# pku-lab-1806-llm/lab-1806-vec-db

Hardware: AMD Instinct MI355X
Metric: queries/sec at recall@10, Gist1M d=960 (Flat brute force, L2Sqr, k=10) (higher is better)
Workload: dtype f32 (int8 lower-bound filter pass); 1 GPU; flat_knn_gist1m; rows=1000000, dim=960, k=10, dist=L2Sqr, parallelism=single GPU, steps_in_flight=1, queries_per_corpus_pass=128

## Files before the change

lab_1806_vec_db_amd/csrc/api.hip:

```cpp
#include <algorithm>
#include <cmath>
#include <cstring>

#include "ctx.hpp"
#include "pq_hnsw.hpp"

using namespace vdb;

static thread_local std::string g_last_error;
void vdb::set_last_error(const std::string &m) { g_last_error = m; }
void vdb::require_gpu() {
    int cnt = 0;
    hipError_t e = hipGetDeviceCount(&cnt);
    if (e != hipSuccess || cnt <= 0)
        throw Error(VDB_ERR_NOGPU, std::string("no usable HIP device (libvdbhip has no CPU fallback): ") +
                                       hipGetErrorString(e));
}

void vdb::merge_topk_dev(Index &ix, const void *d_dists, const void *d_ids, const void *d_counts, uint64_t stride_d,
                           uint64_t stride_i, uint64_t stride_c, uint64_t n_shards, uint64_t nq, uint64_t k,
                           void *d_out_idx, void *d_out_dist, void *d_out_count, void *stream) {
    VDB_REQUIRE(d_dists && d_ids && d_counts && d_out_idx && d_out_dist && d_out_count, "null argument");
    VDB_REQUIRE(k >= 1 && k <= 1024, "k must be in 1..1024");
    VDB_REQUIRE(nq <= 65535 && n_shards <= 65535, "too many queries or shards for one call");
// ... 536 lines not shown
    else if (n == "flat_gemm_tw")
        gemm_set_tw((int)value);
    else if (n == "flat_gemm_nt")
        gemm_set_nt((int)value);
    else if (n == "flat_gemm_zigzag")
        gemm_set_zigzag((int)value);
    else if (n == "flat_gemm_block_rows") {
        VDB_REQUIRE(value >= 0, "flat_gemm_block_rows must be >= 0");
        gemm_set_block_rows((uint64_t)value);
    }
    else if (n == "flat_gemm_stagger")
        gemm_set_stagger((int)value);
    else if (n == "flat_gemm_debug")
        idx->ix.flat_gemm_debug = (int)value;
    else if (n == "flat_tail")
        idx->ix.flat_tail_mode = (int)value;
    else if (n == "flat_tail_lb_nw")
        flat_tail_lb_set_nw((int)value);
    else if (n == "flat_small")
        idx->ix.flat_small_mode = (int)value;
    else if (n == "flat_small_max_rows")
        idx->ix.flat_small_max_rows = (uint64_t)value;
    else if (n == "flat_half")
        idx->ix.flat_half_mode = (int)value;
    else if (n == "flat_i8")
        idx->ix.flat_i8_mode = (int)value;
    else if (n == "flat_i8_rows") {
        VDB_REQUIRE(value >= 64 && value <= 8192 && value % 64 == 0, "flat_i8_rows must be a multiple of 64 in [64, 8192]");
        idx->ix.flat_i8_kprime = (uint32_t)value;
    }
    else if (n == "flat_range_max_results") {
        VDB_REQUIRE(value >= 0, "flat_range_max_results must be >= 0");
        idx->ix.range_max_results = (uint64_t)value;
    }
    else if (n == "debug_alloc_fail_over")
        devbuf_fail_over() = (size_t)value;
    else if (n == "flat_i8_unit_min")
        idx->ix.flat_i8_unit_min = (int)value;
    else if (n == "flat_i8_full")
        idx->ix.flat_i8_full = (int)value;
    else if (n == "flat_i8_refine") {
        idx->ix.flat_i8_refine = (int)value;
        idx->ix.i8_refine_on = 0;
        idx->ix.i8_refine_calls = 0;
    }
    else if (n == "flat_i8_second")
        idx->ix.flat_i8_second = (int)value;
    else if (n == "flat_i8_stats") {
        idx->ix.flat_i8_stats = (int)value;
        for (auto &h : idx->ix.i8_rounds_hist) h = 0;
        idx->ix.i8_hits_sum = 0;
        idx->ix.i8_hits_max = 0;
        idx->ix.i8_stat_queries = 0;
    }
    else if (n == "flat_i8_hits") {
        VDB_REQUIRE(value >= 256 && value <= 4096, "flat_i8_hits must be in [256, 4096]");
        idx->ix.flat_i8_hits = (uint32_t)value;
    }
    else if (n == "flat_gemm8_sample_res")
        gemm8_set_sample_res((int)value);
    else if (n == "flat_gemm8_nt")
        gemm8_set_nt((int)value);
    else if (n == "flat_gemm8_kc")
        gemm8_set_kc((int)value);
    else if (n == "flat_gemm8_burst")
        gemm8_set_burst((int)value);
    else if (n == "flat_gemm8_res")
        gemm8_set_res((int)value);
    else if (n == "flat_gemm8_coop")
        gemm8_set_coop((int)value);
    else if (n == "flat_gemm8_grid")
        gemm8_set_grid((int)value);
    else if (n == "flat_gemm_coop")
        gemm_set_coop((int)value);
    else if (n == "flat_half_kmul") {
        VDB_REQUIRE(value >= 1 && value <= 64, "flat_half_kmul must be in [1, 64]");
        idx->ix.flat_half_kmul = (uint32_t)value;
    }
    else
        throw Error(VDB_ERR_INVALID, "unknown parameter " + n);
    VDB_API_END
}
int vdb_index_prepare(vdb_index *idx, int all_tiers) {
    VDB_API_BEGIN
    VDB_REQUIRE(idx, "null index");
    require_gpu();
    idx->ix.prepare_flat(all_tiers != 0);
    VDB_API_END
}
int vdb_flat_fallback_count(const vdb_index *idx, uint64_t *out) {
    VDB_API_BEGIN
    VDB_REQUIRE(idx && out, "null argument");
    *out = idx->ix.fallback_count.load();
    VDB_API_END
}

int vdb_get_stat(const vdb_index *idx, const char *name, uint64_t *out) {
    VDB_API_BEGIN
    VDB_REQUIRE(idx && name && out, "null argument");
    std::string n(name);
    if (n == "flat_fallback")
        *out = idx->ix.fallback_count.load();
    else if (n == "flat_half_queries")
        *out = idx->ix.half_queries.load();
    else if (n == "flat_half_redo")
        *out = idx->ix.half_redo.load();
    else if (n == "flat_half_valid")
        *out = idx->ix.half_m.valid ? 1 : 0;
    else if (n == "flat_gemm_coop_sets")
        *out = gemm_last_coop();
    else if (n == "flat_gemm8_coop_sets")
        *out = gemm8_last_coop();
    else if (n == "flat_i8_queries")
        *out = idx->ix.i8_queries.load();
    else if (n == "flat_i8_redo")
        *out = idx->ix.i8_redo.load();
    else if (n == "flat_i8_valid")
        *out = idx->ix.i8_m.valid ? 1 : 0;
    else if (n == "flat_range_queries")
        *out = idx->ix.range_queries.load();
    else if (n == "flat_range_i8_queries")
        *out = idx->ix.range_i8_queries.load();
    else if (n == "flat_range_scan_queries")
        *out = idx->ix.range_scan_queries.load();
    else if (n == "flat_range_hits")
        *out = idx->ix.range_hits.load();
    else if (n == "flat_range_hits_max")
        *out = idx->ix.range_hits_max.load();
    else if (n == "flat_range_results")
        *out = idx->ix.range_results.load();
    else if (n.rfind("flat_i8_rounds_", 0) == 0 && n.size() == 16 && n[15] >= '0' && n[15] <= '8')
        *out = idx->ix.i8_rounds_hist[n[15] - '0'].load();
    else if (n == "mirror_alloc_failures")
        *out = idx->ix.mirror_alloc_failures.load();
    else if (n == "flat_i8_second_queries")
        *out = idx->ix.i8_second_queries.load();
    else if (n == "flat_i8_second_redo")
        *out = idx->ix.i8_second_redo.load();
    else if (n == "flat_i8_hits_sum")
        *out = idx->ix.i8_hits_sum.load();
    else if (n == "flat_i8_hits_max")
        *out = idx->ix.i8_hits_max.load();
    else if (n == "flat_i8_stat_queries")
        *out = idx->ix.i8_stat_queries.load();
    else if (n == "flat_i8_rows_walked")
        *out = idx->ix.i8_rows_walked.load();
    else if (n == "flat_bf16_mirror")
        *out = idx->ix.tiled_built ? 1 : 0;
    else if (n == "hnsw_heap_walk_queries")
        *out = idx->ix.hnsw.heap_walk_queries.load();
    else if (n == "hnsw_half_dropped")
        *out = idx->ix.hnsw.last_half_dropped.load();
    else if (n == "ivf_last_offers")
        *out = idx->ix.ivf.last_offers.load();
    else if (n == "ivf_last_rows_fetched_q8")
        *out = idx->ix.ivf.last_rows_fetched_q8.load();
    else if (n == "ivf_last_kept_q8")
        *out = idx->ix.ivf.last_kept_q8.load();
    else if (n == "ivf_last_kept")
        *out = idx->ix.ivf.last_kept.load();
    else if (n == "pq_adc16_queries")
        *out = idx->ix.pq.adc16_queries.load();
    else if (n == "pq_adc16_redo")
        *out = idx->ix.pq.adc16_redo.load();
    else if (n == "flat_i8_refine_queries")
        *out = idx->ix.i8_refine_queries.load();
    else if (n == "flat_i8_refine_on")
        *out = (uint64_t)idx->ix.i8_refine_on.load();
    else if (n == "pq_q8_overflow")
        *out = idx->ix.pq.q8_overflow.load();
    else if (n == "pq_q8_short")
        *out = idx->ix.pq.q8_short.load();
    else if (n == "pq_q8_hits_sum")
        *out = idx->ix.pq.q8_hits_sum.load();
    else if (n == "pq_q8_hits_max")
        *out = idx->ix.pq.q8_hits_max.load();
    else if (n == "hbm_bytes_per_row")
        *out = idx->ix.hbm_bytes_per_row();
    else
        throw Error(VDB_ERR_INVALID, "unknown statistic " + n);
    VDB_API_END
}

int vdb_pq_attach(vdb_index *idx, uint64_t n_bits, uint64_t m, const float *centroids, const uint8_t *codes) {
    VDB_API_BEGIN
    VDB_REQUIRE(idx && centroids, "null argument");
    pq_attach(idx->ix, n_bits, m, centroids, codes);
    VDB_API_END
}
int vdb_pq_build(vdb_index *idx, uint64_t n_bits, uint64_t m, uint64_t train_n, uint64_t max_iter, float tol,
                 uint64_t seed) {
    VDB_API_BEGIN
    VDB_REQUIRE(idx, "null index");
    pq_build(idx->ix, n_bits, m, train_n, max_iter, tol, seed);
    VDB_API_END
}
int vdb_pq_clear(vdb_index *idx) {
// ... 534 lines not shown
```

lab_1806_vec_db_amd/csrc/index.hip:

```cpp
#include "index.hpp"

#include <algorithm>
#include <cmath>
#include <cstring>

namespace vdb {

Index::Index(int dev, uint64_t d, int ds, bool u8) : device(dev), dim(d), dist(ds), elem_u8(u8) {
#ifndef VDB_HOST_SANITIZER_BUILD
    use_device();
    hipDeviceProp_t prop;
    VDB_HIP(hipGetDeviceProperties(&prop, dev));
    num_cu = prop.multiProcessorCount > 0 ? prop.multiProcessorCount : 256;
    std::string arch = prop.gcnArchName;
    if (arch.rfind("gfx950", 0) != 0)
        throw Error(4, "libvdbhip is built for gfx950 (MI355X) only; device reports " + arch);
#endif
}

std::unique_ptr<Workspace> Index::acquire_ws() {
    use_device();
    {
        std::lock_guard<std::mutex> g(ws_mu);
        if (!ws_free.empty()) {
// ... 605 lines not shown
                                 d_cand, d_hits, CAND_CAP, flat_gemm_debug, num_cu, s,
                                 i8_second ? CAND_CAP : std::max<uint32_t>(64u, s_step * s_rank));
    else if (gemm)
        launch_flat_gemm_filter(xt, n, (uint32_t)dim, ws.qfrag_g.as<float>(), d_qmul, (uint32_t)ngroups,
                                d_sq.as<float>(), cosine, d_tau, d_cand, d_hits, CAND_CAP, flat_gemm_debug, num_cu, s);
    else
        launch_flat_mfma_filter(d_tiled.as<float>(), n, (uint32_t)dim, ws.qfrag.as<float>(), (uint32_t)nbatch,
                                d_sq.as<float>(), cosine, d_tau, d_cand, d_hits, CAND_CAP, d_sync, num_cu, s);
    prof_end(ws);
    {
        std::lock_guard<std::mutex> g(pass_mu);
        if (!pass_ev) VDB_HIP(hipEventCreateWithFlags(&pass_ev, hipEventDisableTiming));
        VDB_HIP(hipEventRecord(pass_ev, s));
        pass_ev_valid = true;
    }
    SplitErr se;
    if (half) {
        se.qerr = d_qerr;
        se.dx_abs = half_dx_abs;
        se.dx_rel = half_dx_rel;
    }
    if (i8) {
        se.qoff = d_qoff;
        se.mu_norm = i8_mu_norm;
    }
    if (i8 || (flat_tail_mode != 1 && !elem_u8 && flat_tail64_supported((uint32_t)dim, kprime, ksel))) {
        FlatTailArgs t{};
        t.cand = d_cand;
        t.cap = CAND_CAP;
        t.cnt = d_hits;
        t.kprime = kprime;
        t.ksel = ksel;
        t.kstride = (uint32_t)k;
        t.X = d_rows.as<float>();
        t.dim = (uint32_t)dim;
        t.Q = d_q;
        t.metric = cosine ? MET_COSINE : MET_L2_DIRECT;
        t.xsq = d_sq.as<float>();
        t.qsq = ws.qsq.as<float>();
        t.n_rows = n;
        t.xsq_max = xsq_max;
        t.xsq_min_pos = xsq_min_pos;
        t.cosine = cosine;
        t.se = se;
        t.id_offset = id_offset;
        bool refine = false;
        if (i8 && !i8_second && nq >= 64 && flat_i8_refine != 1) {
            bool on = flat_i8_refine == 2;
            if (flat_i8_refine == 0 && i8_refine_on.load() != 0) on = (i8_refine_calls.fetch_add(1) % 32u) != 31u;
            refine = on && ensure_rows_h(ws);
        }
        const size_t st_off = (nq + 15) & ~size_t(15);
        const bool want_stats = i8 && flat_i8_stats;
        t.flags = static_cast<uint8_t *>(ws.pinned(want_stats ? st_off + nq * sizeof(uint32_t) : nq));
        if (want_stats) t.qstat = reinterpret_cast<uint32_t *>(t.flags + st_off);
        p.stats = want_stats;
        p.refined = refine;
        if (refine) {
            launch_flat_refine_half(d_rows_h.as<uint16_t>(), (uint32_t)dim, half_sx(), half_dx_abs, half_dx_rel, cosine, d_q, d_sq.as<float>(),
                                    ws.qsq.as<float>(), d_qoff, d_cand, CAND_CAP, d_hits, (uint32_t)nq, CAND_CAP, s);
            i8_refine_queries += nq;
        }
        t.out_idx = d_idx;
        t.out_dist = d_dist;
        t.out_count = d_cnt;
        t.tau = d_tau;
        if (i8 && i8_second && nq <= 96 && flat_i8_full != 1) {
            ws.keys_b.reserve(nq * size_t(CAND_CAP) * sizeof(uint64_t));
            launch_flat_full_lb(t, (uint32_t)nq, ws.keys_b.as<uint64_t>(), ws.keys_c.as<uint64_t>(), s);
        } else if (i8)
            launch_flat_tail_lb(t, (uint32_t)nq, s);
        else
            launch_flat_tail64(t, (uint32_t)nq, s);
    } else {
        launch_topk_merge_counted(d_cand, CAND_CAP, d_hits, (uint32_t)nq, kprime, ws.keys_a.as<uint64_t>(), s);
        rerank_rows((uint32_t)dim, d_q, (uint32_t)nq, cosine ? MET_COSINE : MET_L2_DIRECT, d_sq.as<float>(),
                      ws.qsq.as<float>(), ws.keys_a.as<uint64_t>(), ws.keys_b.as<uint64_t>(), kprime, capp, s);
        launch_topk_merge(ws.keys_b.as<uint64_t>(), 1, capp, (uint32_t)nq, ksel, ws.keys_c.as<uint64_t>(), s);
        launch_flat_finish(ws.keys_c.as<uint64_t>(), capk, ws.keys_a.as<uint64_t>(), capp, (uint32_t)nq, ksel, (uint32_t)k, kprime,
                           n, ws.qsq.as<float>(), xsq_max, xsq_min_pos, cosine, (uint32_t)dim, se, d_hits, CAND_CAP, id_offset,
                           static_cast<uint8_t *>(ws.pinned(nq)), d_idx, d_dist, d_cnt, s);
    }
    p.active = true;
    p.half = half;
    p.i8 = i8;
    p.i8_second = i8_second;
    p.kprime = kprime;
    p.ksel = ksel;
    p.nq = nq;
    p.k = k;
    p.d_q = d_q;
    p.d_idx = d_idx;
    p.d_dist = d_dist;
    p.d_cnt = d_cnt;
}

uint64_t Index::flat_knn_finish(Workspace &ws, FlatPending &p) {
    hipStream_t s = ws.stream;
    if (!p.active) return 0;
    p.active = false;
    const uint64_t nq = p.nq, k = p.k;
    const uint8_t *flags = static_cast<const uint8_t *>(ws.pinned(nq));
    VDB_SYNC(s);
    std::vector<uint64_t> redo;
    for (uint64_t q = 0; q < nq; q++)
        if (flags[q] & 1u) redo.push_back(q);
    if (p.half) {
        half_queries += nq;
        half_redo += redo.size();
    }
    if (p.i8 && p.i8_second) {
        i8_second_queries += nq;
        i8_second_redo += redo.size();
    }
    const bool try_second = p.i8 && !p.i8_second && flat_i8_second != 1 && !redo.empty();
    if (p.i8 && !p.i8_second) {
        i8_queries += nq;
        if (!try_second) i8_redo += redo.size();
        if (flat_i8_refine == 0 && nq >= 64) {
            uint64_t rs = 0;
            for (uint64_t q = 0; q < nq; q++) rs += std::min<uint32_t>(flags[q] >> 1, 32u);
            const double mean_rounds = double(rs) / double(nq);
            if (!p.refined) {
                const int was = i8_refine_on.load();
                const int now = was ? (mean_rounds >= 4.0 ? 1 : 0) : (mean_rounds >= 6.0 ? 1 : 0);
                if (now != was) {
                    i8_refine_on = now;
                    i8_refine_calls = 0;
                }
            }
        }
        if (p.stats) {
            const uint32_t *qs = reinterpret_cast<const uint32_t *>(flags + ((nq + 15) & ~size_t(15)));
            uint64_t hs = 0, hm = 0;
            for (uint64_t q = 0; q < nq; q++) {
                const uint32_t r = qs[q] & 0xFFu, h = qs[q] >> 8;
                i8_rounds_hist[r < 8 ? r : 8] += 1;
                hs += h;
                hm = std::max<uint64_t>(hm, h);
            }
            i8_hits_sum += hs;
            i8_stat_queries += nq;
            uint64_t cur = i8_hits_max.load();
            while (hm > cur && !i8_hits_max.compare_exchange_weak(cur, hm)) {
            }
        }
    }
    if (redo.empty()) return 0;
    if (!p.half && !p.i8) fallback_count += redo.size();
    const uint64_t nr = redo.size();
    DevBuf rx, rq, rqs, ri, rd, rc, rdk;
    rx.reserve(nr * sizeof(uint64_t));
    rq.reserve(nr * dim * sizeof(float));
    rqs.reserve(nr * sizeof(float));
    ri.reserve(nr * k * sizeof(uint64_t));
    rd.reserve(nr * k * sizeof(float));
    rc.reserve(nr * sizeof(uint64_t));
    VDB_HIP(hipMemcpyAsync(rx.p, redo.data(), nr * sizeof(uint64_t), hipMemcpyHostToDevice, s));
    launch_gather_rows_f32(p.d_q, rx.as<uint64_t>(), nr, (uint32_t)dim, rq.as<float>(), s);
    launch_gather_rows_f32(ws.qsq.as<float>(), rx.as<uint64_t>(), nr, 1, rqs.as<float>(), s);
    if (try_second) {
        rdk.reserve(nr * sizeof(float));
        launch_gather_dk(p.d_dist, p.d_cnt, rx.as<uint64_t>(), nr, (uint32_t)k, p.ksel, rdk.as<float>(), s);
    }
    VDB_HIP(hipMemsetAsync(ri.p, 0, nr * k * sizeof(uint64_t), s));
    VDB_HIP(hipMemsetAsync(rd.p, 0, nr * k * sizeof(float), s));
    VDB_SYNC(s);
    if (try_second)
        i8_redo += flat_knn_device(ws, rq.as<float>(), nr, k, ri.as<uint64_t>(), rd.as<float>(), rc.as<uint64_t>(), true, 0, true, rdk.as<float>());
    else if (p.i8)
        flat_knn_device(ws, rq.as<float>(), nr, k, ri.as<uint64_t>(), rd.as<float>(), rc.as<uint64_t>(), true, 0, false);
    else if (p.half)
        flat_knn_device(ws, rq.as<float>(), nr, k, ri.as<uint64_t>(), rd.as<float>(), rc.as<uint64_t>(), false, p.kprime);
    else
        flat_exact_device(ws, rq.as<float>(), rqs.as<float>(), nr, p.ksel, k, ri.as<uint64_t>(), rd.as<float>(), rc.as<uint64_t>());
    launch_scatter_results(ri.as<uint64_t>(), rd.as<float>(), rc.as<uint64_t>(), rx.as<uint64_t>(), nr, (uint32_t)k, p.d_idx, p.d_dist, p.d_cnt, s);
    VDB_SYNC(s);
    return p.i8 ? nr : 0;
}

void Index::flat_range_device(Workspace &ws, const float *d_q, uint64_t nq, const float *d_radius, uint64_t limit, RangeResult &out) {
    hipStream_t s = ws.stream;
    out.device = device;
    out.nq = nq;
    out.lims.assign(nq + 1, 0);
    range_queries += nq;
    if (nq == 0) return;
    if (n == 0) {
        range_scan_queries += nq;
        return;
    }
    constexpr uint32_t CAND_CAP = 8192;
    constexpr uint64_t QCH = 1024;
    constexpr uint32_t BQ = 8;
// ... 237 lines not shown
```

lab_1806_vec_db_amd/csrc/index.hpp:

```cpp
#pragma once
#include <algorithm>
#include <atomic>
#include <cmath>
#include <cstdlib>
#include <functional>
#include <map>
#include <memory>
#include <mutex>
#include <string>
#include <vector>

#include "common.hpp"
#include "kernels.hpp"

namespace vdb {

inline bool devbuf_efence() {
    static const bool on = [] {
        const char *e = std::getenv("VDB_EFENCE");
        return e && e[0] == '1';
    }();
    return on;
}
inline std::atomic<size_t> &devbuf_fail_over() {
// ... 224 lines not shown
    size_t elem_size() const { return elem_u8 ? 1 : sizeof(float); }
    const float *rows_f32_view(DevBuf &scratch, uint64_t r0, uint64_t r1, hipStream_t s) const;
    template <class F>
    void for_tile_chunks(Workspace &ws, uint64_t t_begin, uint64_t t_end, uint64_t n_rows, F fn) const {
        if (!elem_u8) {
            fn(d_rows.as<float>(), t_begin, t_end, std::min(t_begin * 16, n_rows), n_rows);
            return;
        }
        constexpr uint64_t CH = 12 * 64;
        ws.dense.reserve(CH * 16 * dim * sizeof(float));
        for (uint64_t t = t_begin; t < t_end; t += CH) {
            const uint64_t tb = std::min(t_end, t + CH), ra = std::min(t * 16, n_rows), rb = std::min(tb * 16, n_rows);
            fn(rows_f32_view(ws.dense, ra, rb, ws.stream), t, tb, ra, rb);
        }
    }
    DevBuf d_rows, d_sq;
    std::atomic<uint64_t> mirror_alloc_failures{0};
    DevBuf d_tiled;
    RowMirror tiled_m{mirror_alloc_failures, {&d_tiled}};
    const std::atomic<bool> &tiled_built = tiled_m.valid;
    bool ensure_tiled(Workspace &ws);
    void prepare_flat(bool all_tiers);
    uint64_t hbm_bytes_per_row() const;
    DevBuf d_tiled_h, d_half_err;
    int half_exp = 0;
    float half_dx_abs = 0.0f, half_dx_rel = 0.0f;
    int flat_half_mode = 0;
    uint32_t flat_half_kmul = 4;
    std::atomic<uint64_t> half_queries{0}, half_redo{0};
    void half_refresh(Workspace &ws, uint64_t n_old, uint64_t n_new);
    RowMirror half_m{mirror_alloc_failures, {&d_tiled_h}};
    bool i8_defers_half() const;
    bool ensure_half(Workspace &ws);
    float half_sx() const { return std::ldexp(1.0f, 13 - half_exp); }
    DevBuf d_tiled_i8, d_rowc_i8, d_mu_i8;
    RowMirror i8_m{mirror_alloc_failures, {&d_tiled_i8, &d_rowc_i8}};
    uint64_t i8_mu_rows = 0;
    float i8_l1 = 0.0f, i8_l2 = 0.0f, i8_mu_norm = 0.0f;
    int flat_i8_mode = 0;
    uint32_t flat_i8_kprime = 2048;
    int flat_i8_full = 0;
    int flat_i8_refine = 0;
    std::atomic<int> i8_refine_on{0};
    std::atomic<uint32_t> i8_refine_calls{0};
    std::atomic<uint64_t> i8_refine_queries{0};
    int flat_i8_unit_min = 0;
    int flat_i8_second = 0;
    std::atomic<uint64_t> i8_second_queries{0}, i8_second_redo{0};
    uint32_t flat_i8_hits = 1024;
    std::atomic<uint64_t> i8_queries{0}, i8_redo{0};
    int flat_i8_stats = 0;
    std::atomic<uint64_t> i8_rounds_hist[9] = {};
    std::atomic<uint64_t> i8_hits_sum{0}, i8_hits_max{0}, i8_stat_queries{0};
    std::atomic<uint64_t> i8_rows_walked{0};
    bool i8_applicable(uint32_t ksel) const;
    bool i8_mirror_applicable() const;
    bool ensure_i8(Workspace &ws);
    void build_i8(Workspace &ws);
    DevBuf d_rows_h;
    RowMirror rows_h_m{mirror_alloc_failures, {&d_rows_h}};
    int rows_h_exp = 0;
    bool ensure_rows_h(Workspace &ws);
    DevBuf d_rows_q8, d_q8_scale, d_q8_err;
    RowMirror rows_q8_m{mirror_alloc_failures, {&d_rows_q8, &d_q8_scale, &d_q8_err}};
    bool ensure_rows_q8(Workspace &ws);
    std::vector<float> h_sq;
    float xsq_max = 0.0f;
    float xsq_min_pos = 3.4e38f;
    mutable std::vector<float> h_rows;
    mutable bool host_valid = true;
    mutable std::mutex host_mu;
    int flat_mode = 0;
    int flat_gemm_mode = 0;
    int flat_gemm_debug = 0;
    int flat_tail_mode = 0;
    int flat_small_mode = 0;
    uint64_t flat_small_max_rows = 16384;
    bool flat_small_applies(uint64_t nq, uint64_t k) const;
    void flat_small_device(Workspace &ws, const float *q, uint64_t nq, uint64_t k, uint64_t *o_idx, float *o_dist, uint64_t *o_cnt);
    std::atomic<uint64_t> fallback_count{0};
    PQState pq;
    HNSWState hnsw;
    IVFState ivf;

    std::mutex ws_mu;
    std::vector<std::unique_ptr<Workspace>> ws_free;
    std::mutex pass_mu;
    hipEvent_t pass_ev = nullptr;
    bool pass_ev_valid = false;
    bool prof_on = false;
    std::mutex prof_mu;
    std::map<std::string, ProfEntry> prof;

    Index(int dev, uint64_t d, int ds, bool u8 = false);
    ~Index() {
        if (pass_ev) (void)hipEventDestroy(pass_ev);
    }
    void use_device() const {
#ifndef VDB_HOST_SANITIZER_BUILD
        VDB_HIP(hipSetDevice(device));
#endif
    }
    std::unique_ptr<Workspace> acquire_ws();
    void release_ws(std::unique_ptr<Workspace> ws);
    const float *host_rows() const;

// ... 40 lines not shown
```

lab_1806_vec_db_amd/csrc/k_exact.hip:

```cpp
#include <algorithm>
#include <atomic>
#include <cstdio>
#include <cstdlib>
#include <vector>

#include "common.hpp"
#include "kernels.hpp"

#pragma clang fp contract(off)

namespace vdb {

enum Fold : int { FOLD_L2 = 0, FOLD_DOT = 1 };

template <int FOLD>
__device__ __forceinline__ float fold1(float acc, float x, float q) {
    if (FOLD == FOLD_L2) {
        float df = x - q;
        float sq = df * df;
        return acc + sq;
    } else {
        float p = x * q;
        return acc + p;
    }
// ... 747 lines not shown
        a.out_idx[uint64_t(q) * a.kstride + lane] = ok ? uint64_t(uint32_t(sorted)) + a.id_offset : 0;
        a.out_dist[uint64_t(q) * a.kstride + lane] = ok ? f32_from_orderable(uint32_t(sorted >> 32)) : 0.0f;
    }
    const uint32_t count = __builtin_popcountll(__ballot(ok));
    if (lane == 0) {
        if (a.out_count) a.out_count[q] = count;
        a.flags[q] = flag;
    }
}
bool flat_tail64_supported(uint32_t dim, uint32_t kprime, uint32_t ksel) {
    return (dim & 3) == 0 && dim >= 64 && dim <= 8192 && kprime >= 1 && kprime <= 64 && ksel >= 1 && ksel <= 64;
}
void launch_flat_tail64(const FlatTailArgs &a, uint32_t nq, hipStream_t s) {
    if (nq == 0) return;
    VDB_REQUIRE(flat_tail64_supported(a.dim, a.kprime, a.ksel), "flat_tail64: unsupported shape");
    const size_t lds = (size_t(a.dim / 4) + 4 * 72) * sizeof(float4);
    if (a.metric == MET_L2_DIRECT)
        hipLaunchKernelGGL((k_flat_tail64<FOLD_L2>), dim3(nq), dim3(256), lds, s, a);
    else
        hipLaunchKernelGGL((k_flat_tail64<FOLD_DOT>), dim3(nq), dim3(256), lds, s, a);
    VDB_HIP(hipGetLastError());
}

#define TAIL_LB_AUTO_NW(nq) 40
template <int NW>
__device__ __forceinline__ uint64_t block_top64_above(const uint64_t *__restrict__ src, uint32_t total, uint64_t (*sbest)[64], uint64_t above) {
    const uint32_t lane = threadIdx.x & 63, wave = threadIdx.x >> 6;
    const uint32_t batches = (total + 255) / 256;
    uint64_t best = PAIR_NONE;
    for (uint32_t bt = wave; bt < batches; bt += NW) {
        uint64_t r[4];
#pragma unroll
        for (int u = 0; u < 4; u++) {
            const uint32_t i = (bt * 4 + u) * 64 + lane;
            const uint64_t v = i < total ? src[i] : PAIR_NONE;
            r[u] = v > above ? v : PAIR_NONE;
        }
        const uint64_t tau = __shfl(best, 63);
        uint64_t lo = r[0] < r[1] ? r[0] : r[1], lo2 = r[2] < r[3] ? r[2] : r[3];
        lo = lo < lo2 ? lo : lo2;
        if (__ballot(lo < tau) == 0) continue;
        bitonic_sort_from<2, 4>(r, lane);
        const uint64_t a = merge64(r[0], r[1], lane), b = merge64(r[2], r[3], lane);
        best = merge64(best, merge64(a, b, lane), lane);
    }
    sbest[wave][lane] = best;
    __syncthreads();
    if (wave != 0) return PAIR_NONE;
    uint64_t m = sbest[0][lane];
#pragma unroll
    for (int w = 1; w < NW; w++) m = merge64(m, sbest[w][lane], lane);
    return m;
}
__device__ __forceinline__ uint8_t flat_certify_lb(uint64_t ek, float kappa, uint32_t q, const FlatTailArgs &a) {
    if (ek == PAIR_NONE) return 1;
    const float dk = f32_from_orderable(uint32_t(ek >> 32));
    return flat_lb_excludes(dk, kappa, a.qsq[q], a.se.qoff[q], a.cosine, a.xsq_max, a.xsq_min_pos, a.se.mu_norm, a.dim) ? 0 : 1;
}
template <int FOLD, int NW, int PCD>
__global__ __launch_bounds__(NW * 64, PCD ? 4 : 1) void k_flat_tail_lb(FlatTailArgs a) {
    constexpr bool PC = PCD != 0;
    static_assert(NW == 8 || NW == 4 || NW == 2 || NW == 1, "a stage covers the 64 keys of a round");
    static_assert(!PC || NW == 4, "producer / consumer fold: four waves");
    constexpr int RW = 64 / NW, NP = RW / 8;
    constexpr int DEPTH = PC ? PCD : (NW == 8 ? 8 : (NW == 4 ? 4 : (NW == 2 ? 3 : 2)));
    extern __shared__ float4 ftl_smem[];
    __shared__ uint64_t sbest[NW][64];
    __shared__ uint64_t skeys[64];
    __shared__ uint32_t s_flag;
    const uint32_t q = blockIdx.x, lane = threadIdx.x & 63, wave = threadIdx.x >> 6;
    const uint32_t d4 = a.dim / 4;
    float4 *qs4 = ftl_smem, *tile = ftl_smem + d4 + wave * (RW * 9);
    for (uint32_t i = threadIdx.x; i < d4; i += NW * 64) qs4[i] = reinterpret_cast<const float4 *>(a.Q + uint64_t(q) * a.dim)[i];
    const uint32_t cnt_q = a.cnt[q];
    const uint32_t total = cnt_q <= a.cap ? cnt_q : 0;
    const uint32_t kk = a.ksel;
    const float tau_q = a.tau[q];
    uint64_t run = PAIR_NONE;
    uint64_t above = 0;
    uint8_t flag = 1;
    const uint32_t rounds = cnt_q <= a.cap ? a.kprime / 64 : 0;
#ifdef VDB_TAIL_STAMPS
    uint32_t ns = 0;
#define TAIL_STAMP()                                                                                      \
    do {                                                                                                  \
        if (a.stamps && threadIdx.x == 0 && ns < 30) a.stamps[q * 32 + ns++] = __builtin_readcyclecounter(); \
    } while (0)
#else
#define TAIL_STAMP() do { } while (0)
#endif
    TAIL_STAMP();
    uint32_t rounds_done = 0;
    for (uint32_t rd = 0; rd < rounds; rd++) {
        rounds_done = rd + 1;
        const uint64_t best = block_top64_above<NW>(a.cand + uint64_t(q) * a.cap, total, sbest, above);
        __syncthreads();
        if (wave == 0) sbest[0][lane] = best;
        if (threadIdx.x < 64) skeys[threadIdx.x] = PAIR_NONE;
        __syncthreads();
        TAIL_STAMP();
        uint32_t idx[NP];
        bool live[NP];
#pragma unroll
        for (int i = 0; i < NP; i++) {
            const uint32_t j = wave * RW + 8 * i + (lane >> 3);
            const uint64_t c = sbest[0][j];
            live[i] = c != PAIR_NONE && j < 63;
            idx[i] = live[i] ? uint32_t(c) : 0u;
#if defined(VDB_TAIL_ABLATE) && VDB_TAIL_ABLATE == 1
            idx[i] &= 63u;
#endif
        }
        float acc;
        if constexpr (PC) {
            const bool consumer = wave == (blockIdx.x & 3u);
            acc = pc_rerank_fold<FOLD, DEPTH>(a.X, a.dim, idx, live, qs4, ftl_smem + d4, wave, lane, consumer);
            const uint64_t c = sbest[0][lane];
            if (consumer && c != PAIR_NONE && lane < 63)
                skeys[lane] = pair_key(FOLD == FOLD_L2 ? acc : epilogue(MET_COSINE, acc, a.xsq[uint32_t(c)], a.qsq[q]), uint32_t(c));
        } else {
            if constexpr (NW == 8)
                acc = group_rerank_fold<FOLD, 8>(a.X, a.dim, idx[0], live[0], qs4, tile, lane);
            else
                acc = group_rerank_fold_n<FOLD, DEPTH, RW>(a.X, a.dim, idx, live, qs4, tile, lane);
            const uint32_t j = wave * RW + lane / NW;
            const uint64_t c = sbest[0][j];
            if (c != PAIR_NONE && j < 63 && lane % NW == 0)
                skeys[j] = pair_key(FOLD == FOLD_L2 ? acc : epilogue(MET_COSINE, acc, a.xsq[uint32_t(c)], a.qsq[q]), uint32_t(c));
        }
        __syncthreads();
        TAIL_STAMP();
        if (wave == 0) {
            run = merge64(run, sort64(skeys[lane], lane), lane);
            const uint64_t ek = __shfl(run, kk - 1), nxt = sbest[0][63];
            if (lane == 0) {
                const float kappa = nxt == PAIR_NONE ? tau_q : f32_from_orderable(uint32_t(nxt >> 32));
                s_flag = flat_certify_lb(ek, kappa, q, a) | (nxt == PAIR_NONE ? 2u : 0u);
            }
        }
        __syncthreads();
        TAIL_STAMP();
        const uint32_t f = s_flag;
        if ((f & 1u) == 0) {
            flag = 0;
            break;
        }
        if (f & 2u) break;
        above = sbest[0][62];
        __syncthreads();
    }
#ifdef VDB_TAIL_STAMPS
    if (a.stamps && threadIdx.x == 0) {
        a.stamps[q * 32 + 30] = ns;
        a.stamps[q * 32 + 31] = total;
    }
#endif
    if (wave != 0) return;
    const bool ok = lane < a.ksel && run != PAIR_NONE;
    if (lane < a.ksel) {
        a.out_idx[uint64_t(q) * a.kstride + lane] = ok ? uint64_t(uint32_t(run)) + a.id_offset : 0;
        a.out_dist[uint64_t(q) * a.kstride + lane] = ok ? f32_from_orderable(uint32_t(run >> 32)) : 0.0f;
    }
    const uint32_t count = __builtin_popcountll(__ballot(ok));
    if (lane == 0) {
        if (a.out_count) a.out_count[q] = count;
        a.flags[q] = uint8_t(flag | ((rounds_done < 127u ? rounds_done : 127u) << 1));
        if (a.qstat) a.qstat[q] = rounds_done | ((cnt_q < 0xFFFFFFu ? cnt_q : 0xFFFFFFu) << 8);
    }
}
bool flat_tail_lb_supported(uint32_t dim, uint32_t kprime, uint32_t ksel) {
    return (dim & 3) == 0 && dim >= 64 && dim <= 8192 && kprime >= 64 && kprime % 64 == 0 && kprime <= 8192 && ksel >= 1 && ksel <= 64;
}
static std::atomic<int> g_tail_lb_nw{0};
void flat_tail_lb_set_nw(int v) { g_tail_lb_nw = v; }
#ifdef VDB_TAIL_STAMPS
static void tail_stamps_report(unsigned long long *d, uint32_t nq, hipStream_t s) {
    VDB_SYNC(s);
    std::vector<unsigned long long> h(size_t(nq) * 32);
    VDB_HIP(hipMemcpy(h.data(), d, h.size() * 8, hipMemcpyDeviceToHost));
    VDB_HIP(hipFree(d));
    uint32_t hist[8] = {0}, nr = 0;
    double sel = 0, fold = 0, cert = 0, life = 0;
    for (uint32_t q = 0; q < nq; q++) {
        const unsigned long long *t = &h[size_t(q) * 32];
        const uint32_t ns = (uint32_t)t[30], r = ns ? (ns - 1) / 3 : 0;
        hist[r < 7 ? r : 7]++;
        if (ns) life += double(t[ns - 1] - t[0]);
        for (uint32_t i = 0; i < r; i++, nr++) {
            sel += double(t[1 + 3 * i] - t[3 * i]);
            fold += double(t[2 + 3 * i] - t[1 + 3 * i]);
            cert += double(t[3 + 3 * i] - t[2 + 3 * i]);
        }
    }
    fprintf(stderr, "TAIL_STAMPS nq %u  queries by rounds 0:%u 1:%u 2:%u 3:%u 4:%u 5+:%u  ticks per round: select %.0f fold %.0f merge+certify %.0f  per workgroup %.0f\n",
            nq, hist[0], hist[1], hist[2], hist[3], hist[4], hist[5] + hist[6] + hist[7], sel / (nr ? nr : 1), fold / (nr ? nr : 1),
            cert / (nr ? nr : 1), life / nq);
}
#endif
void launch_flat_tail_lb(const FlatTailArgs &a0, uint32_t nq, hipStream_t s) {
    if (nq == 0) return;
    FlatTailArgs a = a0;
#ifdef VDB_TAIL_STAMPS
    static std::atomic<int> calls{0};
    const char *want = getenv("VDB_TAIL_STAMPS");
    unsigned long long *stamps = nullptr;
    if (want && ++calls == atoi(want)) {
        VDB_HIP(hipMalloc(&stamps, size_t(nq) * 32 * 8));
        VDB_HIP(hipMemset(stamps, 0, size_t(nq) * 32 * 8));
        a.stamps = stamps;
    }
#endif
    VDB_REQUIRE(flat_tail_lb_supported(a.dim, a.kprime, a.ksel) && (a.metric == MET_L2_DIRECT || a.metric == MET_COSINE) && a.se.qoff && a.tau,
                "flat_tail_lb: unsupported shape");
    VDB_REQUIRE((a.metric == MET_COSINE) == (a.cosine != 0) && (a.metric == MET_L2_DIRECT || (a.xsq && a.qsq)), "flat_tail_lb: metric / norms");
    const size_t lds = (size_t(a.dim / 4) + 2 * 64 * 9) * sizeof(float4);
    int nw = g_tail_lb_nw;
    if (nw != 8 && nw != 4 && nw != 2 && nw != 1 && nw != 40 && nw != 41) nw = TAIL_LB_AUTO_NW(nq);
    if (a.metric == MET_COSINE) {
        if (nw == 8)
            hipLaunchKernelGGL((k_flat_tail_lb<FOLD_DOT, 8, 0>), dim3(nq), dim3(512), lds, s, a);
        else if (nw == 41)
            hipLaunchKernelGGL((k_flat_tail_lb<FOLD_DOT, 4, 5>), dim3(nq), dim3(256), lds, s, a);
        else
            hipLaunchKernelGGL((k_flat_tail_lb<FOLD_DOT, 4, 3>), dim3(nq), dim3(256), lds, s, a);
    } else if (nw == 40)
        hipLaunchKernelGGL((k_flat_tail_lb<FOLD_L2, 4, 3>), dim3(nq), dim3(256), lds, s, a);
    else if (nw == 41)
        hipLaunchKernelGGL((k_flat_tail_lb<FOLD_L2, 4, 5>), dim3(nq), dim3(256), lds, s, a);
    else if (nw == 8)
        hipLaunchKernelGGL((k_flat_tail_lb<FOLD_L2, 8, 0>), dim3(nq), dim3(512), lds, s, a);
    else if (nw == 4)
        hipLaunchKernelGGL((k_flat_tail_lb<FOLD_L2, 4, 0>), dim3(nq), dim3(256), lds, s, a);
    else if (nw == 2)
        hipLaunchKernelGGL((k_flat_tail_lb<FOLD_L2, 2, 0>), dim3(nq), dim3(128), lds, s, a);
    else
        hipLaunchKernelGGL((k_flat_tail_lb<FOLD_L2, 1, 0>), dim3(nq), dim3(64), lds, s, a);
    VDB_HIP(hipGetLastError());
#ifdef VDB_TAIL_STAMPS
    if (stamps) tail_stamps_report(stamps, nq, s);
#endif
}

__global__ __launch_bounds__(64) void k_flat_finish_lb(FlatTailArgs a, const uint64_t *__restrict__ exact_sorted, uint32_t lde) {
    const uint32_t q = blockIdx.x, lane = threadIdx.x;
    const uint32_t cnt_q = a.cnt[q];
    const uint64_t e = lane < a.ksel ? exact_sorted[uint64_t(q) * lde + lane] : PAIR_NONE;
    const uint64_t ek = __shfl(e, a.ksel - 1);
    uint8_t flag = 1;
    if (lane == 0 && cnt_q <= a.cap) flag = flat_certify_lb(ek, a.tau[q], q, a);
    const bool ok = lane < a.ksel && e != PAIR_NONE;
    if (lane < a.ksel) {
        a.out_idx[uint64_t(q) * a.kstride + lane] = ok ? uint64_t(uint32_t(e)) + a.id_offset : 0;
        a.out_dist[uint64_t(q) * a.kstride + lane] = ok ? f32_from_orderable(uint32_t(e >> 32)) : 0.0f;
    }
    const uint32_t count = __builtin_popcountll(__ballot(ok));
    if (lane == 0) {
        if (a.out_count) a.out_count[q] = count;
        a.flags[q] = flag;
        if (a.qstat) a.qstat[q] = 0xFFu | ((cnt_q < 0xFFFFFFu ? cnt_q : 0xFFFFFFu) << 8);
    }
}
void launch_flat_full_lb(const FlatTailArgs &a, uint32_t nq, uint64_t *exact_keys , uint64_t *topk ,
                         hipStream_t s) {
    if (nq == 0) return;
    VDB_REQUIRE(a.ksel >= 1 && a.ksel <= 64 && (a.dim & 3) == 0 && a.se.qoff && a.tau, "flat_full_lb: unsupported shape");
    launch_rerank(a.X, a.dim, a.Q, nq, a.metric, a.xsq, a.qsq, a.cand, exact_keys, a.cap, a.cap, s, a.cnt);
    launch_topk_merge_counted(exact_keys, a.cap, a.cnt, nq, a.ksel, topk, s);
    hipLaunchKernelGGL(k_flat_finish_lb, dim3(nq), dim3(64), 0, s, a, topk, topk_capacity(a.ksel));
    VDB_HIP(hipGetLastError());
}

void launch_certify(const uint64_t *exact_sorted, uint32_t lde, const uint64_t *approx_sorted, uint32_t lda,
                    uint32_t nq, uint32_t k, uint32_t kprime, uint64_t n_rows, const float *qsq, float xsq_max,
                    float xsq_min_pos, int cosine, uint32_t dim, uint8_t *flags, hipStream_t s) {
    if (nq == 0) return;
    hipLaunchKernelGGL(k_certify, dim3((nq + 63) / 64), dim3(64), 0, s, exact_sorted, lde, approx_sorted, lda, nq, k,
                       kprime, n_rows, qsq, xsq_max, xsq_min_pos, cosine, dim, flags);
}

}
```

lab_1806_vec_db_amd/csrc/kernels.hpp:

```cpp
#pragma once
#include <hip/hip_runtime.h>

#include <cstdint>

namespace vdb {

enum Metric : int {
    MET_L2_DIRECT = 0,
    MET_COSINE = 1,
    MET_L2_CACHED = 2,
};

void launch_row_sqnorm(const float *X, uint64_t n, uint32_t dim, float *sq, hipStream_t s);
void launch_scan_exact(const float *X, uint64_t n, uint32_t dim, const float *Q, uint32_t nq, int metric,
                       const float *xsq, const float *qsq, float *out, uint64_t ld, bool use_lds, hipStream_t s);
void launch_rerank(const float *X, uint32_t dim, const float *Q, uint32_t nq, int metric, const float *xsq,
                   const float *qsq, const uint64_t *cand, uint64_t *out, uint32_t ncand, uint32_t ldc,
                   hipStream_t s, const uint32_t *cnt = nullptr);
void launch_finalize(const uint64_t *keys, uint32_t ldk, uint32_t nq, uint32_t ksel, uint32_t kstride,
                     uint64_t id_offset, uint64_t *out_idx, float *out_dist, uint64_t *out_count, hipStream_t s);
void launch_iota_keys(uint64_t *rows, uint32_t nq, uint32_t n, uint32_t ld, hipStream_t s);
struct SplitErr {
    const float *qerr = nullptr;
    float dx_abs = 0.0f, dx_rel = 0.0f;
    const float *qoff = nullptr;
    float mu_norm = 0.0f;
};
void launch_flat_finish(const uint64_t *exact_sorted, uint32_t lde, const uint64_t *approx_sorted, uint32_t lda,
                        uint32_t nq, uint32_t ksel, uint32_t kstride, uint32_t kprime, uint64_t n_rows, const float *qsq,
                        float xsq_max, float xsq_min_pos, int cosine, uint32_t dim, SplitErr se, const uint32_t *cnt, uint32_t cap,
                        uint64_t id_offset, uint8_t *flags, uint64_t *out_idx, float *out_dist, uint64_t *out_count,
                        hipStream_t s);
struct FlatTailArgs {
    const uint64_t *cand;
    uint32_t cap;
    const uint32_t *cnt;
    uint32_t kprime, ksel, kstride;
    const float *X;
    uint32_t dim;
    const float *Q;
    int metric;
    const float *xsq, *qsq;
    uint64_t n_rows;
    float xsq_max, xsq_min_pos;
    int cosine;
    SplitErr se;
    uint64_t id_offset;
    uint8_t *flags;
    uint64_t *out_idx;
    float *out_dist;
    uint64_t *out_count;
    unsigned long long *stamps = nullptr;
    const float *tau = nullptr;
    uint32_t *qstat = nullptr;
};
bool flat_tail_lb_supported(uint32_t dim, uint32_t kprime, uint32_t ksel);
void launch_flat_tail_lb(const FlatTailArgs &a, uint32_t nq, hipStream_t s);
void launch_flat_full_lb(const FlatTailArgs &a, uint32_t nq, uint64_t *exact_keys, uint64_t *topk, hipStream_t s);
void flat_tail_lb_set_nw(int v);
bool flat_tail64_supported(uint32_t dim, uint32_t kprime, uint32_t ksel);
void launch_flat_tail64(const FlatTailArgs &a, uint32_t nq, hipStream_t s);
struct FlatSmallArgs {
    const float *X;
    uint64_t n;
    uint32_t dim;
    const float *Q;
    int metric;
    const float *xsq;
    uint64_t *part;
    uint32_t *counter;
    uint32_t ksel, kstride;
    uint64_t id_offset;
    uint64_t *out_idx;
    float *out_dist;
    uint64_t *out_count;
};
bool flat_small_supported(uint64_t n, uint32_t dim, uint64_t nq, uint64_t k);
uint32_t flat_small_rows_per_wg(uint64_t n, int num_cu);
size_t flat_small_part_keys(uint64_t n, uint64_t nq, uint32_t ksel, int num_cu);
void launch_flat_small(const FlatSmallArgs &a, uint32_t nq, int num_cu, hipStream_t s);
void launch_certify(const uint64_t *exact_sorted, uint32_t lde, const uint64_t *approx_sorted, uint32_t lda,
                    uint32_t nq, uint32_t k, uint32_t kprime, uint64_t n_rows, const float *qsq, float xsq_max,
                    float xsq_min_pos, int cosine, uint32_t dim, uint8_t *flags, hipStream_t s);

void launch_extract_tau(const uint64_t *sorted, uint32_t ld, uint32_t nq, uint32_t kprime, float *tau, hipStream_t s);
void launch_flag_overflow(const uint32_t *cnt, uint32_t cap, uint32_t min_hits, uint32_t nq, uint8_t *flags,
                          hipStream_t s);

uint32_t topk_chunk(uint64_t n);
uint32_t topk_num_lists(uint64_t n);
void launch_select_tau(const float *keys, uint64_t ld, uint32_t n, uint32_t nq, uint32_t nq_real, uint32_t kth, float *tau,
                       hipStream_t s);
uint32_t select_tau_max_n();
uint32_t topk_capacity(uint32_t k);
void launch_topk_dense(const float *keys, uint64_t ld, uint64_t n, uint32_t nq, uint32_t k, uint64_t *lists,
                       hipStream_t s);
void launch_topk_merge(const uint64_t *lists, uint32_t nlists, uint32_t cap_in, uint32_t nq, uint32_t k,
                       uint64_t *out, hipStream_t s);

void launch_topk_merge_counted(const uint64_t *lists, uint32_t cap_in, const uint32_t *cnt, uint32_t nq, uint32_t k,
                               uint64_t *out, hipStream_t s);
void launch_merge_shards64(const float *dists, const uint64_t *ids, const uint64_t *counts, uint64_t stride_d,
                           uint64_t stride_i, uint64_t stride_c, uint32_t S, uint32_t nq, uint32_t k, uint64_t *out_idx,
                           float *out_dist, uint64_t *out_count, hipStream_t s);
void launch_pack_pairs(const float *dists, const uint64_t *ids, const uint64_t *counts, uint64_t stride_d,
                       uint64_t stride_i, uint64_t stride_c , uint32_t S, uint32_t nq, uint32_t k,
                       uint32_t cap_in, uint64_t *lists, hipStream_t s);
// ... 126 lines not shown
```

Before: 1.061 million queries/s.

## Skip fetching tail candidates whose int8 lower bound already exceeds current k-th distance

In the int8 lower-bound tail rerank kernel, each round now checks candidates against the current k-th exact distance and drops those the lower bound already excludes, so their fp32 rows are not fetched or reranked. Dead lanes are remapped to live rows to keep loads uniform, and the certification kappa and restart point are adjusted to the first dropped candidate. The aim is to cut fp32 row fetches in the refinement tail, at the cost of extra ballot and mask logic and possible extra restart rounds. A toggle and stats counters for fetched rows and restarts are also added.

```diff
diff --git a/lab_1806_vec_db_amd/csrc/api.hip b/lab_1806_vec_db_amd/csrc/api.hip
--- a/lab_1806_vec_db_amd/csrc/api.hip
+++ b/lab_1806_vec_db_amd/csrc/api.hip
@@ -612,7 +612,11 @@
         idx->ix.i8_hits_sum = 0;
         idx->ix.i8_hits_max = 0;
         idx->ix.i8_stat_queries = 0;
-    }
+        idx->ix.i8_rows_fetched = 0;
+        idx->ix.i8_tail_restarts = 0;
+    }
+    else if (n == "flat_i8_tail_skip")
+        idx->ix.flat_i8_tail_skip = (int)value;
     else if (n == "flat_i8_hits") {
         VDB_REQUIRE(value >= 256 && value <= 4096, "flat_i8_hits must be in [256, 4096]");
         idx->ix.flat_i8_hits = (uint32_t)value;
@@ -703,6 +707,10 @@
         *out = idx->ix.i8_hits_max.load();
     else if (n == "flat_i8_stat_queries")
         *out = idx->ix.i8_stat_queries.load();
+    else if (n == "flat_i8_rows_fetched")
+        *out = idx->ix.i8_rows_fetched.load();
+    else if (n == "flat_i8_tail_restarts")
+        *out = idx->ix.i8_tail_restarts.load();
     else if (n == "flat_i8_rows_walked")
         *out = idx->ix.i8_rows_walked.load();
     else if (n == "flat_bf16_mirror")
diff --git a/lab_1806_vec_db_amd/csrc/index.hip b/lab_1806_vec_db_amd/csrc/index.hip
--- a/lab_1806_vec_db_amd/csrc/index.hip
+++ b/lab_1806_vec_db_amd/csrc/index.hip
@@ -681,8 +681,12 @@
         }
         const size_t st_off = (nq + 15) & ~size_t(15);
         const bool want_stats = i8 && flat_i8_stats;
-        t.flags = static_cast<uint8_t *>(ws.pinned(want_stats ? st_off + nq * sizeof(uint32_t) : nq));
-        if (want_stats) t.qstat = reinterpret_cast<uint32_t *>(t.flags + st_off);
+        t.flags = static_cast<uint8_t *>(ws.pinned(want_stats ? st_off + 2 * nq * sizeof(uint32_t) : nq));
+        if (want_stats) {
+            t.qstat = reinterpret_cast<uint32_t *>(t.flags + st_off);
+            t.qstat2 = t.qstat + nq;
+        }
+        t.skip = flat_i8_tail_skip != 1 ? 1u : 0u;
         p.stats = want_stats;
         p.refined = refine;
         if (refine) {
@@ -761,14 +765,18 @@
         }
         if (p.stats) {
             const uint32_t *qs = reinterpret_cast<const uint32_t *>(flags + ((nq + 15) & ~size_t(15)));
-            uint64_t hs = 0, hm = 0;
+            uint64_t hs = 0, hm = 0, fs = 0, rs2 = 0;
             for (uint64_t q = 0; q < nq; q++) {
                 const uint32_t r = qs[q] & 0xFFu, h = qs[q] >> 8;
                 i8_rounds_hist[r < 8 ? r : 8] += 1;
                 hs += h;
                 hm = std::max<uint64_t>(hm, h);
+                fs += qs[nq + q] & 0xFFFFFFu;
+                rs2 += qs[nq + q] >> 24;
             }
             i8_hits_sum += hs;
+            i8_rows_fetched += fs;
+            i8_tail_restarts += rs2;
             i8_stat_queries += nq;
             uint64_t cur = i8_hits_max.load();
             while (hm > cur && !i8_hits_max.compare_exchange_weak(cur, hm)) {
diff --git a/lab_1806_vec_db_amd/csrc/index.hpp b/lab_1806_vec_db_amd/csrc/index.hpp
--- a/lab_1806_vec_db_amd/csrc/index.hpp
+++ b/lab_1806_vec_db_amd/csrc/index.hpp
@@ -300,6 +300,9 @@
     int flat_i8_stats = 0;
     std::atomic<uint64_t> i8_rounds_hist[9] = {};
     std::atomic<uint64_t> i8_hits_sum{0}, i8_hits_max{0}, i8_stat_queries{0};
+    std::atomic<uint64_t> i8_rows_fetched{0};
+    std::atomic<uint64_t> i8_tail_restarts{0};
+    int flat_i8_tail_skip = 0;
     std::atomic<uint64_t> i8_rows_walked{0};
     bool i8_applicable(uint32_t ksel) const;
     bool i8_mirror_applicable() const;
diff --git a/lab_1806_vec_db_amd/csrc/k_exact.hip b/lab_1806_vec_db_amd/csrc/k_exact.hip
--- a/lab_1806_vec_db_amd/csrc/k_exact.hip
+++ b/lab_1806_vec_db_amd/csrc/k_exact.hip
@@ -823,10 +823,15 @@
     for (int w = 1; w < NW; w++) m = merge64(m, sbest[w][lane], lane);
     return m;
 }
+__device__ __forceinline__ bool flat_tail_excludes(float dk, float kappa, float qsq_q, float qoff_q, const FlatTailArgs &a) {
+    return flat_lb_excludes(dk, kappa, qsq_q, qoff_q, a.cosine, a.xsq_max, a.xsq_min_pos, a.se.mu_norm, a.dim);
+}
+__device__ __forceinline__ uint8_t flat_certify_lb(uint64_t ek, float kappa, float qsq_q, float qoff_q, const FlatTailArgs &a) {
+    if (ek == PAIR_NONE) return 1;
+    return flat_tail_excludes(f32_from_orderable(uint32_t(ek >> 32)), kappa, qsq_q, qoff_q, a) ? 0 : 1;
+}
 __device__ __forceinline__ uint8_t flat_certify_lb(uint64_t ek, float kappa, uint32_t q, const FlatTailArgs &a) {
-    if (ek == PAIR_NONE) return 1;
-    const float dk = f32_from_orderable(uint32_t(ek >> 32));
-    return flat_lb_excludes(dk, kappa, a.qsq[q], a.se.qoff[q], a.cosine, a.xsq_max, a.xsq_min_pos, a.se.mu_norm, a.dim) ? 0 : 1;
+    return flat_certify_lb(ek, kappa, a.qsq[q], a.se.qoff[q], a);
 }
 template <int FOLD, int NW, int PCD>
 __global__ __launch_bounds__(NW * 64, PCD ? 4 : 1) void k_flat_tail_lb(FlatTailArgs a) {
@@ -839,6 +844,8 @@
     __shared__ uint64_t sbest[NW][64];
     __shared__ uint64_t skeys[64];
     __shared__ uint32_t s_flag;
+    __shared__ uint64_t s_live, s_dead;
+    __shared__ float s_qc[2];
     const uint32_t q = blockIdx.x, lane = threadIdx.x & 63, wave = threadIdx.x >> 6;
     const uint32_t d4 = a.dim / 4;
     float4 *qs4 = ftl_smem, *tile = ftl_smem + d4 + wave * (RW * 9);
@@ -847,6 +854,11 @@
     const uint32_t total = cnt_q <= a.cap ? cnt_q : 0;
     const uint32_t kk = a.ksel;
     const float tau_q = a.tau[q];
+    if (threadIdx.x == 0) {
+        s_qc[0] = a.qsq[q];
+        s_qc[1] = a.se.qoff[q];
+    }
+    uint32_t fetched = 0, restarts = 0;
     uint64_t run = PAIR_NONE;
     uint64_t above = 0;
     uint8_t flag = 1;
@@ -866,18 +878,43 @@
         rounds_done = rd + 1;
         const uint64_t best = block_top64_above<NW>(a.cand + uint64_t(q) * a.cap, total, sbest, above);
         __syncthreads();
-        if (wave == 0) sbest[0][lane] = best;
+        if (wave == 0) {
+            sbest[0][lane] = best;
+            const bool have = best != PAIR_NONE && lane < 63;
+            const uint64_t ek0 = __shfl(run, kk - 1);
+            const bool excl = a.skip && have && ek0 != PAIR_NONE &&
+                              flat_tail_excludes(f32_from_orderable(uint32_t(ek0 >> 32)), f32_from_orderable(uint32_t(best >> 32)), s_qc[0], s_qc[1], a);
+            const uint64_t keep = __ballot(have && !excl);
+            const bool dead = excl && (keep >> lane) == 0;
+            const uint64_t lm_w = __ballot(have && !dead), dm_w = __ballot(dead);
+            if (lane == 0) {
+                s_live = lm_w;
+                s_dead = dm_w;
+            }
+        }
         if (threadIdx.x < 64) skeys[threadIdx.x] = PAIR_NONE;
         __syncthreads();
         TAIL_STAMP();
+        auto uniform64 = [](uint64_t v) -> uint64_t {
+            const uint32_t lo = uint32_t(__builtin_amdgcn_readfirstlane(int(uint32_t(v)))), hi = uint32_t(__builtin_amdgcn_readfirstlane(int(uint32_t(v >> 32))));
+            return uint64_t(lo) | (uint64_t(hi) << 32);
+        };
+        const uint64_t lm = uniform64(s_live), dm = uniform64(s_dead);
+        fetched += __builtin_popcountll(lm);
         uint32_t idx[NP];
         bool live[NP];
 #pragma unroll
         for (int i = 0; i < NP; i++) {
             const uint32_t j = wave * RW + 8 * i + (lane >> 3);
-            const uint64_t c = sbest[0][j];
-            live[i] = c != PAIR_NONE && j < 63;
-            idx[i] = live[i] ? uint32_t(c) : 0u;
+            live[i] = (lm >> j) & 1u;
+            uint32_t js = j;
+            if (!live[i]) {
+                const uint32_t b8 = j & ~7u, bw = wave * RW;
+                const uint64_t m8 = (lm >> b8) & 0xFFull, mw = RW == 64 ? lm : (lm >> bw) & ((1ull << (RW & 63)) - 1ull);
+                js = m8 ? b8 + __builtin_ctzll(m8) : (mw ? bw + __builtin_ctzll(mw) : (lm ? __builtin_ctzll(lm) : 64u));
+            }
+            const uint64_t cs = sbest[0][js & 63u];
+            idx[i] = js < 64u && cs != PAIR_NONE ? uint32_t(cs) : 0u;
 #if defined(VDB_TAIL_ABLATE) && VDB_TAIL_ABLATE == 1
             idx[i] &= 63u;
 #endif
@@ -887,7 +924,7 @@
             const bool consumer = wave == (blockIdx.x & 3u);
             acc = pc_rerank_fold<FOLD, DEPTH>(a.X, a.dim, idx, live, qs4, ftl_smem + d4, wave, lane, consumer);
             const uint64_t c = sbest[0][lane];
-            if (consumer && c != PAIR_NONE && lane < 63)
+            if (consumer && ((lm >> lane) & 1u))
                 skeys[lane] = pair_key(FOLD == FOLD_L2 ? acc : epilogue(MET_COSINE, acc, a.xsq[uint32_t(c)], a.qsq[q]), uint32_t(c));
         } else {
             if constexpr (NW == 8)
@@ -896,7 +933,7 @@
                 acc = group_rerank_fold_n<FOLD, DEPTH, RW>(a.X, a.dim, idx, live, qs4, tile, lane);
             const uint32_t j = wave * RW + lane / NW;
             const uint64_t c = sbest[0][j];
-            if (c != PAIR_NONE && j < 63 && lane % NW == 0)
+            if (((lm >> j) & 1u) && lane % NW == 0)
                 skeys[j] = pair_key(FOLD == FOLD_L2 ? acc : epilogue(MET_COSINE, acc, a.xsq[uint32_t(c)], a.qsq[q]), uint32_t(c));
         }
         __syncthreads();
@@ -905,8 +942,12 @@
             run = merge64(run, sort64(skeys[lane], lane), lane);
             const uint64_t ek = __shfl(run, kk - 1), nxt = sbest[0][63];
             if (lane == 0) {
-                const float kappa = nxt == PAIR_NONE ? tau_q : f32_from_orderable(uint32_t(nxt >> 32));
-                s_flag = flat_certify_lb(ek, kappa, q, a) | (nxt == PAIR_NONE ? 2u : 0u);
+                float kappa = nxt == PAIR_NONE ? tau_q : f32_from_orderable(uint32_t(nxt >> 32));
+                if (dm) {
+                    const float ks = f32_from_orderable(uint32_t(sbest[0][__builtin_ctzll(dm)] >> 32));
+                    kappa = ks < kappa ? ks : kappa;
+                }
+                s_flag = flat_certify_lb(ek, kappa, s_qc[0], s_qc[1], a) | (nxt == PAIR_NONE && dm == 0 ? 2u : 0u);
             }
         }
         __syncthreads();
@@ -917,7 +958,12 @@
             break;
         }
         if (f & 2u) break;
-        above = sbest[0][62];
+        if (dm) {
+            const uint32_t p0 = __builtin_ctzll(dm);
+            if (p0) above = sbest[0][p0 - 1];
+            restarts++;
+        } else
+            above = sbest[0][62];
         __syncthreads();
     }
 #ifdef VDB_TAIL_STAMPS
@@ -937,6 +983,7 @@
         if (a.out_count) a.out_count[q] = count;
         a.flags[q] = uint8_t(flag | ((rounds_done < 127u ? rounds_done : 127u) << 1));
         if (a.qstat) a.qstat[q] = rounds_done | ((cnt_q < 0xFFFFFFu ? cnt_q : 0xFFFFFFu) << 8);
+        if (a.qstat2) a.qstat2[q] = (fetched < 0xFFFFFFu ? fetched : 0xFFFFFFu) | ((restarts < 255u ? restarts : 255u) << 24);
     }
 }
 bool flat_tail_lb_supported(uint32_t dim, uint32_t kprime, uint32_t ksel) {
@@ -1029,6 +1076,7 @@
         if (a.out_count) a.out_count[q] = count;
         a.flags[q] = flag;
         if (a.qstat) a.qstat[q] = 0xFFu | ((cnt_q < 0xFFFFFFu ? cnt_q : 0xFFFFFFu) << 8);
+        if (a.qstat2) a.qstat2[q] = 0;
     }
 }
 void launch_flat_full_lb(const FlatTailArgs &a, uint32_t nq, uint64_t *exact_keys , uint64_t *topk ,
diff --git a/lab_1806_vec_db_amd/csrc/kernels.hpp b/lab_1806_vec_db_amd/csrc/kernels.hpp
--- a/lab_1806_vec_db_amd/csrc/kernels.hpp
+++ b/lab_1806_vec_db_amd/csrc/kernels.hpp
@@ -53,6 +53,8 @@
     unsigned long long *stamps = nullptr;
     const float *tau = nullptr;
     uint32_t *qstat = nullptr;
+    uint32_t *qstat2 = nullptr;
+    uint32_t skip = 1;
 };
 bool flat_tail_lb_supported(uint32_t dim, uint32_t kprime, uint32_t ksel);
 void launch_flat_tail_lb(const FlatTailArgs &a, uint32_t nq, hipStream_t s);
```

New measurement: 1.061 million queries/s (median of 2 runs). No clear change (+0.0%).
